# ergodicio/tsadar

Measured on AMD Instinct MI355X. Metric: spectra/sec (fwd+grad), 1024-lambda EPW+IAW form factor, batch 4096, higher is better.
Workload: dtype f64

## Files before the change

tsadar_amd/csrc/k_spectrum_fused.inc:

```

#ifdef TSFF_TRACE
__device__ unsigned long long* g_trace_buf = nullptr;
#define TSFF_STAMP(k) do { if (tid == 0 && g_trace_buf) g_trace_buf[(size_t)item * 16 + (k)] = wall_clock64(); } while (0)
#define TSFF_STAMP_WAVE(k) do { if (lane == 0 && g_trace_buf) g_trace_buf[(size_t)item * 16 + (k) + hw] = wall_clock64(); } while (0)
#define TSFF_STAMP_HW() do { if (tid == 0 && g_trace_buf) g_trace_buf[(size_t)item * 16] = ((unsigned long long)__builtin_amdgcn_s_getreg(20 | (31 << 11)) << 32) | (unsigned)__builtin_amdgcn_s_getreg(4 | (31 << 11)); } while (0)
#else
#define TSFF_STAMP(k) do {} while (0)
#define TSFF_STAMP_WAVE(k) do {} while (0)
#define TSFF_STAMP_HW() do {} while (0)
#endif

constexpr int kRedSums = 32;
template <int NI, int GM, bool ZH, bool EX = false>
__global__ __launch_bounds__(kHalf, 2) void k_spectrum_fused(KStatic S, KCall K, int f0, int flags,
                                                             const double* __restrict__ lrec) {
  const bool use_ks = flags & kFlagKsCache, interleaved = flags & kFlagInterleaved;
  const int item = blockIdx.x;
  const int f_il = interleaved ? (int)(item >= K.B) : 0;
  const int b = K.b0 + item - f_il * K.B, tid = threadIdx.x;
  const size_t gitem = (size_t)f_il * K.Btot + b;
  constexpr int TPF = kHalf, NW = TPF / 64;
  constexpr bool PAD = kSelectFree<NI>;
  const int ht = tid, lane = tid & 63, hw = tid >> 6;
  const int f = __builtin_amdgcn_readfirstlane(interleaved ? f_il : f0);
  extern __shared__ __align__(16) unsigned char smem[];
  TSFF_STAMP_HW();
  TSFF_STAMP(1);
  const Smem m = carve(smem, S, 1, GM, use_ks, true, ZH, EX);
  constexpr int NPk = TSFF_NP(NI);
  const double* __restrict__ xpar = K.params + (size_t)b * S.NP;
  const int npts = S.npts, NA = S.n_angles;
  const int hs = S.hs, Ls = npts / 4 + 2 * hs;
  double* xs = m.x;
  auto XA = [&](int j) { return (j & 3) * Ls + (j >> 2) + hs; };
  Tables T;
  const double lam_shift = S.lam_shift[f];
  const double* __restrict__ omgs = S.omgs[f];
  const int jp[2] = {kPair * ht, npts / 2 + kPair * ht};
  double ws[2][kPair + 1];
  LineS<NI> L;
  double* __restrict__ ksc = use_ks ? m.ksc : nullptr;
  {
    TSFF_STAGE_LOCALS;
    stage_issue(TSFF_STAGE_ARGS, m, S, K, S.shared_fe ? 0 : b, ZH, f);
    stage_commit(TSFF_STAGE_ARGS, m, S, K, S.shared_fe ? 0 : b, T, ZH, f, PAD);
#pragma unroll
    for (int p = 0; p < 2; ++p)
#pragma unroll
      for (int q = 0; q <= kPair; ++q) ws[p][q] = omgs[min(jp[p] + q, npts - 1)];
    {
      lines_load<NI>(lrec + gitem * kLineRec, 1, [](double v) { return uni(v); }, L);
    }
    if (use_ks) ks_cache_fill(ksc, jp, ws, L.wpe2, npts);
    zero_phase_halos(xs, Ls, hs, ht, TPF);
  }
  double w_lo[2], w_hi[2];
#pragma unroll
  for (int p = 0; p < 2; ++p) {
    w_lo[p] = lane_f64(ws[p][0], 0);
    w_hi[p] = lane_f64(ws[p][kPair], 63);
  }
  const bool far0 = far_range_w<NI>(w_lo[0], w_hi[0], L), far1 = far_range_w<NI>(w_lo[1], w_hi[1], L);
  const double ex_wse = ((lane >> 4) & 1) ? w_hi[1] : w_hi[0];
  __syncthreads();
  TSFF_STAMP(2);
  auto JQ = [&](int q) { return jp[q >> 1] + (q & 1); };
  LineS<NI> J[kStrip];
  KsAcc KA[kStrip];
  double xa[kStrip];
#pragma unroll
  for (int q = 0; q < kStrip; ++q) { zero_lines<NI>(J[q]); xa[q] = 0.0; KA[q].p1a = KA[q].p2a = KA[q].p1b = KA[q].p2b = 0.0; }
  const double cw = -0.5 * L.i2wL * L.i2wL;
  double* exb = m.ex;
  if (EX) {
    const int Pb = (lane >> 4) & 1, ab = lane & 15;
    if (lane < 32 && ab < NA) unit_boundary_fill<NI, PAD>(ex_wse, m.cosa[ab], L, T, exb + 16 * (2 * hw + Pb) + ab);
    __builtin_amdgcn_fence(__ATOMIC_RELEASE, "wavefront");
    __builtin_amdgcn_wave_barrier();
    __builtin_amdgcn_fence(__ATOMIC_ACQUIRE, "wavefront");
  }
  cdouble_t* arp = (cdouble_t*)(lrec + (size_t)K.Btot * (interleaved ? 2 : 1) * kLineRec + gitem * 2 * (size_t)NA);
  auto sweep = [&](auto pair_tag, auto far_tag) {
    constexpr int P = decltype(pair_tag)::value;
    constexpr bool FAR = decltype(far_tag)::value;
    const int jb = jp[P];
    const int j2 = min(jb + kPair, npts - 1);
    const double ks2 = EX ? (use_ks ? ksc[j2] : ks_eval(ws[P][kPair], L.wpe2)) : 0.0;
    cdouble_t* pn = arp;
    double ct_n = pn[0], wa_n = pn[1];
    const double* exu = EX ? exb + 16 * (2 * hw + P) : nullptr;
    double ksa = 0.0, ksb = 0.0;
    if constexpr (kSweepSched<NI, GM, ZH, EX>) {
      ksa = use_ks ? ksc[jb] : ks_eval(ws[P][0], L.wpe2);
      ksb = use_ks ? ksc[min(jb + 1, npts - 1)] : ks_eval(ws[P][1], L.wpe2);
    }
    for (int a = 0; a < NA; ++a) {
      const double ct = ct_n, wa = wa_n;
      { pn += a + 1 < NA ? 2 : 0; ct_n = pn[0]; wa_n = pn[1]; }
      if constexpr (kSweepSched<NI, GM, ZH, EX>) {
        constexpr int q0 = kPair * P;
        static_assert(kPair == 2, "pair_step_sched is written out for two points");
        pair_step_sched<NI, GM, ZH, FAR, PAD>(ws[P], ksa, ksb, ks2, exu + a, pair_has_next<NI, P, 2>(1, jb + 1, npts), L, T, ct, wa, cw,
                                              xa[q0], J[q0], KA[q0], xa[q0 + 1], J[q0 + 1], KA[q0 + 1]);
        continue;
      }
      Base b0;
      base_eval<NI, PAD>(ws[P][0], use_ks ? ksc[jb] : ks_eval(ws[P][0], L.wpe2), ct, L, T, b0);
      const Base b0f = b0;
#pragma unroll
      for (int i = 0; i < kPair; ++i) {
        constexpr int q0 = kPair * P;
        const int q = q0 + i, j = jb + i;
        const bool has_next = pair_has_next<NI, P, 2>(i, j, npts);
        Base b1;
        if (EX && i == kPair - 1) {
          neighbour_take<NI>(b0f, exu + a, ks2, ct, L, b1);
        } else {
          base_eval<NI, PAD>(ws[P][i + 1], use_ks ? ksc[min(j + 1, npts - 1)] : ks_eval(ws[P][i + 1], L.wpe2), ct, L, T, b1);
        }
        row_step<NI, GM, ZH, FAR, PAD>(b0, b1, has_next, L, T, ct, wa, cw, xa[q], J[q], KA[q]);
        b0 = b1;
      }
    }
  };
  if (far0) sweep(std::integral_constant<int, 0>{}, std::true_type{}); else sweep(std::integral_constant<int, 0>{}, std::false_type{});
  if (far1) sweep(std::integral_constant<int, 1>{}, std::true_type{}); else sweep(std::integral_constant<int, 1>{}, std::false_type{});
  TSFF_STAMP_WAVE(9);
#pragma unroll
  for (int q = 0; q < kStrip; ++q) {
    const int j = JQ(q);
    const double ksa = use_ks ? ksc[j] : ks_eval(ws[q >> 1][q & 1], L.wpe2);
    const double ksb = use_ks ? ksc[min(j + 1, npts - 1)] : ks_eval(ws[q >> 1][(q & 1) + 1], L.wpe2);
    ks_columns<NI>(KA[q], ksa, ksb, L, J[q]);
  }
  {
    const bool filt = f == TSFF_FEATURE_ELE && S.filt;
#pragma unroll
    for (int q = 0; q < kStrip; ++q) store_scaled(xs + XA(JQ(q)), xa[q], ws[q >> 1][q & 1], filt, S.filt, JQ(q));
  }
  __syncthreads();
  TSFF_STAMP(3);

  constexpr int BPT = 4;
  const bool raw = S.raw[f];
  const size_t row4 = (size_t)b * TSFF_NBINS + 4 * ht;
  double dpre[BPT], npre[BPT], lpre[BPT];
  uint8_t mpre[BPT];
#pragma unroll
  for (int r = 0; r < BPT; ++r) {
    dpre[r] = K.data[f][row4 + r];
    npre[r] = K.noise[f] ? K.noise[f][row4 + r] : 0.0;
    lpre[r] = f == TSFF_FEATURE_ELE ? S.lam_bin[f][4 * ht + r] : 0.0;
    mpre[r] = S.mask[f][4 * ht + r];
  }
  const double amps = raw ? 1.0 : K.amps[f][b];
  const double* __restrict__ lrp = lrec + gitem * kLineRec + 9 + 4 * NI;
  const double p_lam_v = lrp[0], p_amp1_v = lrp[1], p_amp2_v = lrp[2], p_amp3_v = lrp[3];
  double wpre[BPT];
  {
    const bool filt = f == TSFF_FEATURE_ELE && S.filt;
#pragma unroll
    for (int r = 0; r < BPT; ++r) {
      const double w = omgs[4 * ht + r];
      wpre[r] = filt ? w * w * S.filt[4 * ht + r] : w * w;
    }
  }
  double ybin[BPT] = {0.0, 0.0, 0.0, 0.0};
  conv4_phase<1>(xs, Ls, ht + S.cf_a0[f] + hs, (cdouble_t*)(S.ptaps[f] + S.cf_i0[f]), S.cf_na[f], ybin);
  double M = ybin[0];
  int pstar = 4 * ht;
#pragma unroll
  for (int r = 1; r < BPT; ++r)
    if (ybin[r] > M) { M = ybin[r]; pstar = 4 * ht + r; }
  half_argmax<NW>(M, pstar, m.red, 0, hw, lane);
  TSFF_STAMP(4);
  const double invM = raw ? 1.0 : 1.0 / M;
  const double p_lam = uni(p_lam_v), p_amp1 = uni(p_amp1_v), p_amp2 = uni(p_amp2_v), p_amp3 = uni(p_amp3_v);
  double Tb[BPT], Ap[BPT];
  double s0 = 0.0, s1 = 0.0;
#pragma unroll
  for (int r = 0; r < BPT; ++r) {
    const int pb = 4 * ht + r;
    const double A = bin_amplitude(f, raw, amps, lpre[r], p_lam, p_amp1, p_amp2, p_amp3);
    Ap[r] = A;
    const double t = thry_value(A, ybin[r], invM, K.noise[f] != nullptr, npre[r]);
    if (K.thry[f]) K.thry[f][(size_t)b * TSFF_NBINS + pb] = t;
    Tb[r] = bin_loss(S, K, f, dpre[r], t, mpre[r], s0, s1);
  }

  double sn = 0.0, a1b = 0.0, a2b = 0.0;
#pragma unroll
  for (int r = 0; r < BPT; ++r) norm_adjoint_bin(f, Tb[r], ybin[r], invM, Ap[r], amps, lpre[r], p_lam, sn, a1b, a2b);
  {
    double v5[5] = {s0, s1, sn, a1b, a2b};
#pragma unroll
    for (int k = 0; k < 5; ++k) v5[k] = wave_sum(v5[k]);
    if (lane == 0) {
#pragma unroll
      for (int k = 0; k < 5; ++k) m.red[kRedSums + k * NW + hw] = v5[k];
    }
  }
#pragma unroll
  for (int r = 0; r < BPT; ++r) xs[XA(4 * ht + r)] = Tb[r] * Ap[r] * invM;
  __syncthreads();
  TSFF_STAMP(5);
  double sx[4] = {0.0, 0.0, 0.0, 0.0};
  conv4_phase<-1>(xs, Ls, ht + S.ca_a0[f] + hs, (cdouble_t*)(S.ptaps[f] + S.ca_i0[f]), S.ca_na[f], sx);

  __syncthreads();
  TSFF_STAMP(6);
  {
    const double* r = m.red + kRedSums;
    s0 = (r[0] + r[1]) + (r[2] + r[3]);
    s1 = (r[NW] + r[NW + 1]) + (r[NW + 2] + r[NW + 3]);
    sn = (r[2 * NW] + r[2 * NW + 1]) + (r[2 * NW + 2] + r[2 * NW + 3]);
    a1b = (r[3 * NW] + r[3 * NW + 1]) + (r[3 * NW + 2] + r[3 * NW + 3]);
    a2b = (r[4 * NW] + r[4 * NW + 1]) + (r[4 * NW + 2] + r[4 * NW + 3]);
  }
  if (ht == 0) {
    if (f == TSFF_FEATURE_ELE) { K.lpart[(size_t)b * 3 + 1] = s0; K.lpart[(size_t)b * 3 + 2] = s1; }
    else K.lpart[(size_t)b * 3 + 0] = s0;
  }
  if (raw) sn = a1b = a2b = 0.0;
  {
    const bool filt = f == TSFF_FEATURE_ELE && S.filt;
    const double cn = sn * invM;
    const int s_first = 4 * ht - pstar - S.toff[f], nt = S.ntaps[f];
#pragma unroll
    for (int r = 0; r < 4; ++r) {
      const int i = 4 * ht + r, st = s_first + r;
      const double xb = (st >= 0 && st < nt) ? __builtin_fma(-cn, m.taps[3 + st], sx[r]) : sx[r];
      xs[XA(i)] = xb * wpre[r];
    }
  }
  __syncthreads();
  constexpr int NLB = 9 + 3 * NI;
  LineS<NI> LB;
  zero_lines<NI>(LB);
#pragma unroll
  for (int q = 0; q < kStrip; ++q) {
    const double xb = xs[XA(JQ(q))];
    LB.wpe2 += xb * J[q].wpe2; LB.wL += xb * J[q].wL; LB.kL += xb * J[q].kL; LB.ivTe += xb * J[q].ivTe;
    LB.a_e += xb * J[q].a_e; LB.Ud += xb * J[q].Ud; LB.Vd += xb * J[q].Vd; LB.m += xb * J[q].m;
    LB.pref += xb * xa[q];
#pragma unroll
    for (int s = 0; s < NI; ++s) { LB.ixi[s] += xb * J[q].ixi[s]; LB.a_i[s] += xb * J[q].a_i[s]; LB.cs[s] += xb * J[q].cs[s]; }
  }
  LB.pref *= 1.0 / L.pref;
#pragma unroll
  for (int s = 0; s < NI; ++s) LB.a_i[s] *= -0.5;
  {
    double lb[kLBRec];
    lines_adj_store<NI>(LB, lb);
#pragma unroll
    for (int k = 0; k < NLB; ++k) lb[k] = wave_sum(lb[k]);
    lb[NLB] = a1b; lb[NLB + 1] = a2b;
    const size_t nitems = (size_t)K.Btot * (interleaved ? 2 : 1);
    double mine = 0.0;
#pragma unroll
    for (int k = 0; k < NLB + 2; ++k) mine = lane == k ? lb[k] : mine;
    if (lane < NLB + 2) K.lbrec[((size_t)lane * NW + hw) * nitems + gitem] = mine;
  }
  TSFF_STAMP(8);
}

template <int NI>
__global__ __launch_bounds__(64) void k_fused_prep(KStatic S, const double* __restrict__ params, int B, int f0, int nload,
                                                   double* __restrict__ lrec, double* __restrict__ finrec, double* __restrict__ arec) {
  constexpr int NPk = TSFF_NP(NI);
  const int item = blockIdx.x * 64 + threadIdx.x;
  if (item >= B * nload) return;
  const size_t nitems = (size_t)B * nload;
  const int l = item / B, b = item - l * B, f = nload == 2 ? l : f0;
  const double* __restrict__ x = params + (size_t)b * S.NP;
  double sgv[NPk];
#pragma unroll
  for (int s = 0; s < NPk; ++s) sgv[s] = S.p_sig[s] ? sigmoid(x[s]) : 0.0;
  Phys<NI> p;
  load_phys<NI>(x, S.p_scale, S.p_shift, S.p_sig, S.ti_same, true, p, sgv);
  LineS<NI> L;
  make_lines<NI>(p, S.lam_shift[f], 0, 1, L);
  {
    double ph[NPk + 1];
    phys_to_array<NI>(p, ph);
    double* __restrict__ q = finrec + item;
#pragma unroll
    for (int k = 0; k <= NPk; ++k) q[(size_t)k * nitems] = ph[k];
#pragma unroll
    for (int k = 0; k < NPk; ++k) q[(size_t)(NPk + 1 + k) * nitems] = sgv[k];
    lines_store<NI>(L, q + (size_t)(2 * NPk + 1) * nitems, nitems);
  }
  double* __restrict__ r = lrec + (size_t)item * kLineRec;
  lines_store<NI>(L, r, 1);
  r[9 + 4 * NI] = p.lam; r[10 + 4 * NI] = p.amp1; r[11 + 4 * NI] = p.amp2; r[12 + 4 * NI] = p.amp3;
  if (arec) {
    double2* __restrict__ ar = reinterpret_cast<double2*>(arec) + (size_t)item * S.n_angles;
    for (int a = 0; a < S.n_angles; ++a) ar[a] = make_double2(S.cos_sa[a], S.w_sa[a] * L.pref);
  }
}

template <int NI>
__global__ __launch_bounds__(kThreads) void k_fused_finish(KStatic S, const double* __restrict__ finrec, const double* __restrict__ lbrec,
                                                     const double* __restrict__ lpart, int B, int f0, int nload, int gm,
                                                     const uint8_t* __restrict__ gmask, double* __restrict__ grad,
                                                     double* __restrict__ loss_out, const int* __restrict__ act, int n_act,
                                                     long B_global, long b_off, double* __restrict__ packed) {
  constexpr int NPk = TSFF_NP(NI), NLB = 9 + 3 * NI, NW = kHalf / 64;
  __shared__ double red[8];
  const int lane = threadIdx.x;
  const int per_wg = kThreads / nload;
  if (blockIdx.x == gridDim.x - 1) {
    double a[3] = {0.0, 0.0, 0.0};
    constexpr int U = 8;
    for (int b0 = threadIdx.x; b0 < B; b0 += U * kThreads) {
      double v[U][3];
#pragma unroll
      for (int u = 0; u < U; ++u) {
        const int bb = b0 + u * kThreads;
#pragma unroll
        for (int k = 0; k < 3; ++k) v[u][k] = bb < B ? lpart[(size_t)bb * 3 + k] : 0.0;
      }
#pragma unroll
      for (int u = 0; u < U; ++u)
        if (b0 + u * kThreads < B) { a[0] += v[u][0]; a[1] += v[u][1]; a[2] += v[u][2]; }
    }
    double* out = packed ? packed : loss_out;
    for (int k = 0; k < 3; ++k) {
      const double v = block_sum(a[k], red);
      if (threadIdx.x == 0) out[k] = v;
    }
    return;
  }
  const int b = blockIdx.x * per_wg + lane / nload, l = nload == 2 ? (lane & 1) : 0;
  int actv[NPk];
#pragma unroll
  for (int k = 0; k < NPk; ++k) actv[k] = (packed && k < n_act) ? act[k] : -1;
  const size_t nitems = (size_t)B * nload;
  double gv[NPk];
#pragma unroll
  for (int s = 0; s < NPk; ++s) gv[s] = 0.0;
  if (b < B) {
    const int f = nload == 2 ? l : f0;
    const size_t item = (size_t)l * B + b;
    const double* __restrict__ q = finrec + item;
    double ph[NPk + 1], sgv[NPk];
#pragma unroll
    for (int k = 0; k <= NPk; ++k) ph[k] = q[(size_t)k * nitems];
#pragma unroll
    for (int k = 0; k < NPk; ++k) sgv[k] = q[(size_t)(NPk + 1 + k) * nitems];
    Phys<NI> p;
    phys_from_lds<NI>(ph, p);
    q += (size_t)(2 * NPk + 1) * nitems;
    LineS<NI> L;
    lines_load<NI>(q, nitems, [](double v) { return v; }, L);
    double lb[NLB];
#pragma unroll
    for (int k = 0; k < NLB; ++k) {
      const double* __restrict__ r = lbrec + (size_t)k * NW * nitems + item;
      lb[k] = (r[0] + r[nitems]) + (r[2 * nitems] + r[3 * nitems]);
    }
    const double a1b = lbrec[(size_t)NLB * NW * nitems + item], a2b = lbrec[(size_t)(NLB + 1) * NW * nitems + item];
    LineS<NI> LB;
    zero_lines<NI>(LB);
    lines_adj_load<NI>(lb, true, LB);
    double g[NPk];
#pragma unroll
    for (int s = 0; s < NPk; ++s) g[s] = 0.0;
    make_lines_adjoint<NI>(p, S.lam_shift[f], 0, 1, L, LB, g);
    amp_adjoint(f, a1b, a2b, g);
    tie_renorm_adjoint<NI>(S, p, gm == 1, g);
#pragma unroll
    for (int s = 0; s < NPk; ++s) gv[s] = activation_adjoint(g[s], S.p_scale[s], S.p_sig[s], [&] { return sgv[s]; }, gmask[s]);
  }
  if (nload == 2) {
#pragma unroll
    for (int s = 0; s < NPk; ++s) {
      const double o = __shfl_xor(gv[s], 1, 64);
      gv[s] = (lane & 1) ? 0.0 : gv[s] + o;
    }
  }
  if (b < B && l == 0) {
    if (packed) {
#pragma unroll
      for (int k = 0; k < NPk; ++k) {
        double v = 0.0;
#pragma unroll
        for (int s = 0; s < NPk; ++s) v = actv[k] == s ? gv[s] : v;
        if (actv[k] >= 0) packed[3 + (size_t)k * B_global + b_off + b] = v;
      }
    } else {
#pragma unroll
      for (int s = 0; s < NPk; ++s) grad[(size_t)b * NPk + s] = gv[s];
    }
  }
  if (packed) {
    const long n = (long)n_act * B_global;
    if ((long)B < B_global)
      for (long i = (long)blockIdx.x * kThreads + lane; i < n; i += (long)(gridDim.x - 1) * kThreads) {
        const long k = i / B_global, bl = i - k * B_global - b_off;
        if (bl < 0 || bl >= B) packed[3 + i] = 0.0;
      }
  }
}
```

tsadar_amd/csrc/tsff_device.h:

```cpp
#pragma once
#include <hip/hip_runtime.h>
#include <stdint.h>
#include <type_traits>

#include "../../include/tsff.h"

namespace tsff {

constexpr int kThreads = 256;
constexpr int kStrip = 4;
constexpr int kNP_MAX = TSFF_NP(TSFF_MAX_ION);

enum SpectrumFlag : int {
  kFlagAccumulate = 1,
  kFlagKsCache = 2,
  kFlagInterleaved = 4,
  kFlagOwnScalars = 8,
  kFlagSplit = 16,
};

constexpr double kC = 2.99792458e10;
constexpr double kMe = 510.9896 / (kC * kC);
constexpr double kMp = kMe * 1836.1;
constexpr double kRe = 2.8179e-13;
constexpr double kPi = 3.14159265358979323846;
constexpr double kEsq = kMe * kC * kC * kRe;
constexpr double kC0sq = 4.0 * kPi * kEsq / kMe;
constexpr double kOmgLnum = 2.0 * kPi * 1e7 * kC;
constexpr double kInvSqrt2Pi = 0.39894228040143267794;
constexpr double kSqrt2 = 1.41421356237309504880;

constexpr double kXi2_0 = -8.2;
constexpr double kXi2_h = 0.01;
constexpr double kXi2_ih = 100.0;
constexpr int kNXi2 = TSFF_NXI2;
constexpr int kNXi1 = TSFF_NXI1;

#ifndef TSFF_NEWTON
#define TSFF_NEWTON 1
#endif
__device__ __forceinline__ double frcp(double x) {
  double y = __builtin_amdgcn_rcp(x);
  double e = __builtin_fma(-x, y, 1.0);
  y = __builtin_fma(y, e, y);
#if TSFF_NEWTON > 1
  e = __builtin_fma(-x, y, 1.0);
  y = __builtin_fma(y, e, y);
#endif
  return y;
}

__device__ __forceinline__ void fsqrt2(double x, double& s, double& is) {
  const double y = __builtin_amdgcn_rsq(x);
  double g = x * y, h = 0.5 * y;
  double r = __builtin_fma(-h, g, 0.5);
  g = __builtin_fma(g, r, g);
  h = __builtin_fma(h, r, h);
#if TSFF_NEWTON > 1
  r = __builtin_fma(-h, g, 0.5);
  g = __builtin_fma(g, r, g);
  h = __builtin_fma(h, r, h);
#endif
  const double d = __builtin_fma(-g, g, x);
  s = __builtin_fma(d, h, g);
  is = h + h;
}

__device__ __forceinline__ void fsqrt2_pair(double x0, double x1, double& s0, double& is0, double& s1, double& is1) {
  static_assert(TSFF_NEWTON == 1, "fsqrt2_pair is written out for one refinement step");
  const double y0 = __builtin_amdgcn_rsq(x0), y1 = __builtin_amdgcn_rsq(x1);
  __builtin_amdgcn_sched_barrier(0);
  double g0 = x0 * y0, g1 = x1 * y1, h0 = 0.5 * y0, h1 = 0.5 * y1;
  __builtin_amdgcn_sched_barrier(0);
  const double r0 = __builtin_fma(-h0, g0, 0.5), r1 = __builtin_fma(-h1, g1, 0.5);
  __builtin_amdgcn_sched_barrier(0);
  g0 = __builtin_fma(g0, r0, g0); g1 = __builtin_fma(g1, r1, g1);
  h0 = __builtin_fma(h0, r0, h0); h1 = __builtin_fma(h1, r1, h1);
  __builtin_amdgcn_sched_barrier(0);
  const double d0 = __builtin_fma(-g0, g0, x0), d1 = __builtin_fma(-g1, g1, x1);
  __builtin_amdgcn_sched_barrier(0);
  s0 = __builtin_fma(d0, h0, g0); s1 = __builtin_fma(d1, h1, g1);
  is0 = h0 + h0; is1 = h1 + h1;
}

__device__ __forceinline__ double uni(double x) {
  const int lo = __builtin_amdgcn_readfirstlane(__double2loint(x));
  const int hi = __builtin_amdgcn_readfirstlane(__double2hiint(x));
  return __hiloint2double(hi, lo);
}

__device__ __forceinline__ double next_lane_f64(double v, double last) {
  constexpr int kWaveShl1 = 0x130;
  const int lo = __builtin_amdgcn_update_dpp(__double2loint(last), __double2loint(v), kWaveShl1, 0xf, 0xf, false);
  const int hi = __builtin_amdgcn_update_dpp(__double2hiint(last), __double2hiint(v), kWaveShl1, 0xf, 0xf, false);
  return __hiloint2double(hi, lo);
}

__device__ __forceinline__ double wave_sum(double v) {
#pragma unroll
  for (int o = 32; o > 0; o >>= 1) v += __shfl_xor(v, o, 64);
  return v;
}

__device__ __forceinline__ double block_sum(double v, double* scratch) {
  v = wave_sum(v);
  const int lane = threadIdx.x & 63, w = threadIdx.x >> 6;
  __syncthreads();
  if (lane == 0) scratch[w] = v;
  __syncthreads();
  return (scratch[0] + scratch[1]) + (scratch[2] + scratch[3]);
}

__device__ __forceinline__ void block_argmax(double& v, int& idx, double* scratch) {
#pragma unroll
  for (int o = 32; o > 0; o >>= 1) {
    double ov = __shfl_xor(v, o, 64);
    int oi = __shfl_xor(idx, o, 64);
    if (ov > v || (ov == v && oi < idx)) { v = ov; idx = oi; }
  }
  const int lane = threadIdx.x & 63, w = threadIdx.x >> 6;
  __syncthreads();
  if (lane == 0) { scratch[w] = v; scratch[4 + w] = (double)idx; }
  __syncthreads();
  v = scratch[0]; idx = (int)scratch[4];
#pragma unroll
  for (int k = 1; k < 4; ++k) {
    double ov = scratch[k]; int oi = (int)scratch[4 + k];
    if (ov > v || (ov == v && oi < idx)) { v = ov; idx = oi; }
  }
}

struct Tables {
  const double2* zp;
  const double* W;
  const double2* ht;
  const double2* hc;
  const double2* hcm;
  const double* Wm;
  double* Wb;
  double* Hy;
  double* Hs;
  double vx0, dv, idv, vxlast;
  double u0, utop;
  double uhi;
  const double* etab;
  int nvx;
};
__device__ __forceinline__ void tables_set_grid(Tables& T, double vx0, double dv, int nvx) {
  T.vx0 = vx0; T.dv = dv; T.idv = 1.0 / dv; T.vxlast = vx0 + (nvx - 1) * dv; T.nvx = nvx;
  T.u0 = -vx0 * T.idv; T.utop = (double)(nvx - 1) * (1.0 - 1.1102230246251565e-16); T.uhi = (double)(nvx - 1);
}

struct FeAcc {
  int iw, ih;
  double w0, w1, y0, y1, s0, s1;
};
__device__ __forceinline__ void fe_acc_init(FeAcc& a) { a.iw = a.ih = -1; a.w0 = a.w1 = a.y0 = a.y1 = a.s0 = a.s1 = 0.0; }
__device__ __forceinline__ void fe_flush_w(FeAcc& a, double* Wb) {
  if (a.iw >= 0) { atomicAdd(&Wb[a.iw], a.w0); atomicAdd(&Wb[a.iw + 1], a.w1); }
  a.w0 = a.w1 = 0.0;
}
__device__ __forceinline__ void fe_flush_h(FeAcc& a, double* Hy, double* Hs) {
  if (a.ih >= 0) {
    atomicAdd(&Hy[a.ih], a.y0); atomicAdd(&Hy[a.ih + 1], a.y1);
    atomicAdd(&Hs[a.ih], a.s0); atomicAdd(&Hs[a.ih + 1], a.s1);
  }
  a.y0 = a.y1 = a.s0 = a.s1 = 0.0;
}
__device__ __forceinline__ void fe_add_w(FeAcc& a, double* Wb, double xe, double wb) {
  const double xlast = kXi2_0 + (kNXi2 - 1) * kXi2_h;
  const double u = (xe - kXi2_0) * kXi2_ih;
  int i = (int)u;
  i = i < 0 ? 0 : (i > kNXi2 - 2 ? kNXi2 - 2 : i);
  double t = (xe - (kXi2_0 + i * kXi2_h)) * kXi2_ih;
  t = xe < kXi2_0 ? 0.0 : (xe > xlast ? 1.0 : t);
  if (i != a.iw) { fe_flush_w(a, Wb); a.iw = i; }
  a.w0 += wb * (1.0 - t);
  a.w1 += wb * t;
}
__device__ __forceinline__ void fe_add_h(FeAcc& a, const Tables& T, double x, double hb) {
  if (x < T.vx0 || x > T.vxlast) return;
  const double u = (x - T.vx0) * T.idv;
  int i = (int)u;
  i = i < 0 ? 0 : (i > T.nvx - 2 ? T.nvx - 2 : i);
  const double t = (x - (T.vx0 + i * T.dv)) * T.idv;
  if (i != a.ih) { fe_flush_h(a, T.Hy, T.Hs); a.ih = i; }
  const double t2 = t * t, t3 = t2 * t;
  a.y0 += hb * (2.0 * t3 - 3.0 * t2 + 1.0);
  a.y1 += hb * (3.0 * t2 - 2.0 * t3);
  a.s0 += hb * (t3 - 2.0 * t2 + t) * T.dv;
  a.s1 += hb * (t3 - t2) * T.dv;
}

struct WCell { double a, b, t; bool in; };
__device__ __forceinline__ void w_request(const double* W, double xe, WCell& c) {
#pragma clang fp contract(off)
  constexpr double kTop = (double)(kNXi2 - 1) * (1.0 - 1.1102230246251565e-16);
  const double u = __builtin_fma(xe, kXi2_ih, -kXi2_0 * kXi2_ih);
  const double uc = fmin(fmax(u, 0.0), kTop);
  const double fl = __builtin_floor(uc);
  c.t = uc - fl;
  const int i = (int)fl;
  c.a = W[i]; c.b = W[i + 1];
  c.in = u == uc;
}
__device__ __forceinline__ void w_finish(const WCell& c, double& w, double& dw) {
#pragma clang fp contract(off)
  const double d = c.b - c.a;
  w = __builtin_fma(c.t, d, c.a);
  dw = c.in ? d * kXi2_ih : 0.0;
}
__device__ __forceinline__ void w_lookup(const double* W, double xe, double& w, double& dw) {
  WCell c;
  w_request(W, xe, c);
  w_finish(c, w, dw);
}

__device__ __forceinline__ void hermite_coeffs(double2 a, double2 b, double dv, double2& c01, double2& c23) {
  const double f0 = a.x, f1 = b.x, m0 = a.y * dv, m1 = b.y * dv;
  c01 = make_double2(f0, m0);
  c23 = make_double2(-3.0 * f0 + 3.0 * f1 - 2.0 * m0 - m1, 2.0 * f0 - 2.0 * f1 + m0 + m1);
}

__device__ __forceinline__ void hermite_pad_cell(double2* hc, int nvx, double outside, int tid) {
  if (tid == 0) { hc[2 * (nvx - 1)] = make_double2(outside, 0.0); hc[2 * (nvx - 1) + 1] = make_double2(0.0, 0.0); }
}

struct HCell { double2 c01, c23; double t; bool out; };
template <bool PAD = false>
__device__ __forceinline__ void hermite_request(const Tables& T, double x, HCell& c) {
#pragma clang fp contract(off)
  const double u = __builtin_fma(x, T.idv, T.u0);
  const double uc = PAD ? fmin(fmax(u, -1.0), T.uhi) : fmin(fmax(u, 0.0), T.utop);
  const double fl = __builtin_floor(uc);
  c.t = uc - fl;
  int i = (int)fl;
  if (PAD) { const unsigned iu = (unsigned)i, itop = (unsigned)(T.nvx - 1); i = (int)(iu < itop ? iu : itop); }
  c.c01 = T.hc[2 * i]; c.c23 = T.hc[2 * i + 1];
  c.out = !PAD && u != uc;
}
__device__ __forceinline__ void hermite_finish(const Tables& T, const HCell& c, double& H, double& dH) {
#pragma clang fp contract(off)
  const double t = c.t;
  const double Hi = __builtin_fma(t, __builtin_fma(t, __builtin_fma(t, c.c23.y, c.c23.x), c.c01.y), c.c01.x);
  const double dHi = __builtin_fma(t, __builtin_fma(3.0 * t, c.c23.y, 2.0 * c.c23.x), c.c01.y) * T.idv;
  H = c.out ? -50.0 : Hi;
  dH = c.out ? 0.0 : dHi;
}
template <bool PAD = false>
__device__ __forceinline__ void hermite_lookup_c(const Tables& T, double x, double& H, double& dH) {
  HCell c;
  hermite_request<PAD>(T, x, c);
  hermite_finish(T, c, H, dH);
}

__device__ __forceinline__ void hermite_lookup(const Tables& T, double x, double& H, double& dH) {
  double u = (x - T.vx0) * T.idv;
  int i = (int)u;
  i = i < 0 ? 0 : (i > T.nvx - 2 ? T.nvx - 2 : i);
  const double t = (x - (T.vx0 + i * T.dv)) * T.idv;
  const double2 a = T.ht[i], b = T.ht[i + 1];
  const double f0 = a.x, f1 = b.x, m0 = a.y * T.dv, m1 = b.y * T.dv;
  const double c2 = -3.0 * f0 + 3.0 * f1 - 2.0 * m0 - m1;
  const double c3 = 2.0 * f0 - 2.0 * f1 + m0 + m1;
  if (x < T.vx0 || x > T.vxlast) { H = -50.0; dH = 0.0; }
  else {
    H = f0 + t * (m0 + t * (c2 + t * c3));
    dH = (m0 + t * (2.0 * c2 + 3.0 * t * c3)) * T.idv;
  }
}

template <int NI>
struct Phys {
  double Te, ne, m, lam, amp1, amp2, amp3, neg, teg, ud, Va;
  double Ti[NI], Z[NI], A[NI], fr[NI];
  double fsum;
};

template <int NI>
struct LineS {
  double wpe2, wL, kL, ivTe, a_e, pref, Ud, Vd;
  double i2wL;
  double m;
  double ixi[NI], a_i[NI], cs[NI];
  double hai[NI];
};

__device__ __forceinline__ double grad_coef(int g, int G) {
  return G == 1 ? -1.0 / 200.0 : -1.0 / 200.0 + (double)g / (100.0 * (double)(G - 1));
}

template <int NI>
__device__ __forceinline__ void make_lines(const Phys<NI>& p, double lam_shift, int g, int G, LineS<NI>& L) {
  const double cg = grad_coef(g, G);
  const double ne_g = 1.0e20 * p.ne * (1.0 + p.neg * cg);
  const double Te_g = p.Te * (1.0 + p.teg * cg);
  L.wL = kOmgLnum / (p.lam + lam_shift);
  L.i2wL = 2.0 / L.wL;
  L.m = 0.0;
  L.wpe2 = kC0sq * ne_g;
  L.kL = sqrt(L.wL * L.wL - L.wpe2) / kC;
  L.ivTe = 1.0 / sqrt(Te_g / kMe);
  L.a_e = L.wpe2 * L.ivTe * L.ivTe;
  L.pref = kRe * kRe * ne_g / (2.0 * kPi * kC);
  L.Ud = p.ud * 1e6;
  L.Vd = p.Va * 1e6;
  double Zbar = 0.0;
#pragma unroll
  for (int s = 0; s < NI; ++s) Zbar += p.Z[s] * p.fr[s];
#pragma unroll
  for (int s = 0; s < NI; ++s) {
    const double Ms = p.A[s] * kMp;
    const double vTi = sqrt(p.Ti[s] / Ms);
    L.ixi[s] = 1.0 / (kSqrt2 * vTi);
    L.a_i[s] = kC0sq * kMe * p.Z[s] * p.Z[s] * p.fr[s] * ne_g / (Zbar * p.Ti[s]);
    L.cs[s] = p.fr[s] * p.Z[s] * p.Z[s] / (Zbar * vTi);
    L.hai[s] = -0.5 * L.a_i[s];
  }
}

template <int NI>
__device__ __forceinline__ void make_lines_uniform(const Phys<NI>& p, double lam_shift, int g, int G, LineS<NI>& L) {
  make_lines<NI>(p, lam_shift, g, G, L);
  L.wpe2 = uni(L.wpe2); L.wL = uni(L.wL); L.i2wL = uni(L.i2wL); L.kL = uni(L.kL); L.ivTe = uni(L.ivTe);
  L.a_e = uni(L.a_e); L.pref = uni(L.pref); L.Ud = uni(L.Ud); L.Vd = uni(L.Vd);
#pragma unroll
  for (int s = 0; s < NI; ++s) { L.ixi[s] = uni(L.ixi[s]); L.a_i[s] = uni(L.a_i[s]); L.cs[s] = uni(L.cs[s]); L.hai[s] = uni(L.hai[s]); }
}

template <int NI>
__device__ __forceinline__ void make_lines_adjoint(const Phys<NI>& p, double lam_shift, int g, int G,
                                                   const LineS<NI>& L, const LineS<NI>& LB, double* pb) {
  const double cg = grad_coef(g, G);
  const double gfn = 1.0 + p.neg * cg, gft = 1.0 + p.teg * cg;
  const double ne_g = 1.0e20 * p.ne * gfn;
  const double Te_g = p.Te * gft;
  double wpe2b = LB.wpe2, wLb = LB.wL, ivTeb = LB.ivTe;
  double ne_gb = LB.pref * (kRe * kRe / (2.0 * kPi * kC));
  wpe2b += LB.a_e * L.ivTe * L.ivTe;
  ivTeb += LB.a_e * 2.0 * L.wpe2 * L.ivTe;
  wLb += LB.kL * L.wL / (kC * kC * L.kL);
  wpe2b += LB.kL * (-0.5 / (kC * kC * L.kL));
  double Zbar = 0.0;
#pragma unroll
  for (int s = 0; s < NI; ++s) Zbar += p.Z[s] * p.fr[s];
  double Zbarb = 0.0;
#pragma unroll
  for (int s = 0; s < NI; ++s) {
    const double Ms = p.A[s] * kMp;
    const double vTi = sqrt(p.Ti[s] / Ms);
    const double Z2 = p.Z[s] * p.Z[s];
    double Tib = 0.0, Zb = 0.0, frb = 0.0;
    const double ai_over_fr = kC0sq * kMe * Z2 * ne_g / (Zbar * p.Ti[s]);
    Zb += LB.a_i[s] * 2.0 * L.a_i[s] / p.Z[s];
    frb += LB.a_i[s] * ai_over_fr;
    ne_gb += LB.a_i[s] * L.a_i[s] / ne_g;
    Zbarb -= LB.a_i[s] * L.a_i[s] / Zbar;
    Tib -= LB.a_i[s] * L.a_i[s] / p.Ti[s];
    Tib += LB.ixi[s] * (-0.5 * L.ixi[s] / p.Ti[s]);
    Tib += LB.cs[s] * (-0.5 * L.cs[s] / p.Ti[s]);
    Zb += LB.cs[s] * 2.0 * L.cs[s] / p.Z[s];
    frb += LB.cs[s] * Z2 / (Zbar * vTi);
    Zbarb -= LB.cs[s] * L.cs[s] / Zbar;
    pb[TSFF_P_ION0 + 4 * s + TSFF_ION_TI] += Tib;
    pb[TSFF_P_ION0 + 4 * s + TSFF_ION_Z] += Zb;
    pb[TSFF_P_ION0 + 4 * s + TSFF_ION_FRACT] += frb;
  }
#pragma unroll
  for (int s = 0; s < NI; ++s) {
    pb[TSFF_P_ION0 + 4 * s + TSFF_ION_Z] += Zbarb * p.fr[s];
    pb[TSFF_P_ION0 + 4 * s + TSFF_ION_FRACT] += Zbarb * p.Z[s];
  }
  const double Te_gb = ivTeb * (-0.5 * L.ivTe / Te_g);
  ne_gb += wpe2b * kC0sq;
  const double lam0 = p.lam + lam_shift;
  pb[TSFF_P_LAM] += wLb * (-L.wL / lam0);
  pb[TSFF_P_NE] += ne_gb * 1.0e20 * gfn;
  pb[TSFF_P_NE_GRADIENT] += ne_gb * 1.0e20 * p.ne * cg;
  pb[TSFF_P_TE] += Te_gb * gft;
  pb[TSFF_P_TE_GRADIENT] += Te_gb * p.Te * cg;
  pb[TSFF_P_UD] += LB.Ud * 1e6;
  pb[TSFF_P_VA] += LB.Vd * 1e6;
  pb[TSFF_P_M] += LB.m;
}


template <bool CLAMP = true>
__device__ __forceinline__ double fexp(double x) {
  if (CLAMP) x = fmax(x, -800.0);
  const double n = __builtin_rint(x * 1.4426950408889634074);
  double r = __builtin_fma(n, -6.93147180369123816490e-01, x);
  r = __builtin_fma(n, -1.90821492927058770002e-10, r);
  double p = 1.6059043836821613e-10;
  p = __builtin_fma(p, r, 2.08767569878681e-09);
  p = __builtin_fma(p, r, 2.505210838544172e-08);
  p = __builtin_fma(p, r, 2.755731922398589e-07);
  p = __builtin_fma(p, r, 2.7557319223985893e-06);
  p = __builtin_fma(p, r, 2.48015873015873e-05);
  p = __builtin_fma(p, r, 1.984126984126984e-04);
  p = __builtin_fma(p, r, 1.388888888888889e-03);
  p = __builtin_fma(p, r, 8.333333333333333e-03);
  p = __builtin_fma(p, r, 4.1666666666666664e-02);
  p = __builtin_fma(p, r, 1.6666666666666666e-01);
  p = __builtin_fma(p, r, 0.5);
// ... 556 lines not shown
```

Before: 5.332 million.

## Use scatter-style multi-value wave reductions and reload omega to ease register pressure

Replaces the per-value butterfly wave_sum loops with a recursive halving scatter reduction. Each exchange step sums two values into one using permlane32/16 swaps and DPP, so each lane ends up owning one final sum, with the -0.5 and 1/pref scaling folded into the first step. For the GM==1, NI==1, EX specialisation it also reloads the third omega point from global memory instead of keeping it live in registers across the sweep, and adds asm barriers to stop the compiler from merging the copies. The aim is fewer shuffle instructions in the reductions and lower VGPR pressure, at the cost of extra global loads and more complex lane-ownership logic.

```diff
diff --git a/tsadar_amd/csrc/k_spectrum_fused.inc b/tsadar_amd/csrc/k_spectrum_fused.inc
--- a/tsadar_amd/csrc/k_spectrum_fused.inc
+++ b/tsadar_amd/csrc/k_spectrum_fused.inc
@@ -20,6 +20,7 @@
   const int b = K.b0 + item - f_il * K.B, tid = threadIdx.x;
   const size_t gitem = (size_t)f_il * K.Btot + b;
   constexpr int TPF = kHalf, NW = TPF / 64;
+  constexpr bool kLeanKs = GM == 1 && NI == 1 && EX;
   constexpr bool PAD = kSelectFree<NI>;
   const int ht = tid, lane = tid & 63, hw = tid >> 6;
   const int f = __builtin_amdgcn_readfirstlane(interleaved ? f_il : f0);
@@ -51,7 +52,16 @@
     {
       lines_load<NI>(lrec + gitem * kLineRec, 1, [](double v) { return uni(v); }, L);
     }
-    if (use_ks) ks_cache_fill(ksc, jp, ws, L.wpe2, npts);
+    if constexpr (kLeanKs) {
+      double wsc[2][kPair + 1];
+#pragma unroll
+      for (int p = 0; p < 2; ++p)
+#pragma unroll
+        for (int q = 0; q <= kPair; ++q) { wsc[p][q] = ws[p][q]; asm volatile("" : "+v"(wsc[p][q])); }
+      if (use_ks) ks_cache_fill(ksc, jp, wsc, L.wpe2, npts);
+    } else {
+      if (use_ks) ks_cache_fill(ksc, jp, ws, L.wpe2, npts);
+    }
     zero_phase_halos(xs, Ls, hs, ht, TPF);
   }
   double w_lo[2], w_hi[2];
@@ -60,6 +70,12 @@
     w_lo[p] = lane_f64(ws[p][0], 0);
     w_hi[p] = lane_f64(ws[p][kPair], 63);
   }
+  auto w_third = [&](int p) {
+    const double* o = omgs;
+    int t = ht;
+    asm volatile("" : "+s"(o), "+v"(t));
+    return o[min(kPair * t + p * (npts / 2) + kPair, npts - 1)];
+  };
   const bool far0 = far_range_w<NI>(w_lo[0], w_hi[0], L), far1 = far_range_w<NI>(w_lo[1], w_hi[1], L);
   const double ex_wse = ((lane >> 4) & 1) ? w_hi[1] : w_hi[0];
   __syncthreads();
@@ -85,7 +101,13 @@
     constexpr bool FAR = decltype(far_tag)::value;
     const int jb = jp[P];
     const int j2 = min(jb + kPair, npts - 1);
-    const double ks2 = EX ? (use_ks ? ksc[j2] : ks_eval(ws[P][kPair], L.wpe2)) : 0.0;
+    double wr[kPair + 1];
+    if constexpr (kLeanKs) {
+#pragma unroll
+      for (int q = 0; q <= kPair; ++q) wr[q] = q == kPair ? w_third(P) : ws[P][q];
+    }
+    const double (&wP)[kPair + 1] = [&]() -> const double (&)[kPair + 1] { if constexpr (kLeanKs) return wr; else return ws[P]; }();
+    const double ks2 = EX ? (use_ks ? ksc[j2] : ks_eval(wP[kPair], L.wpe2)) : 0.0;
     cdouble_t* pn = arp;
     double ct_n = pn[0], wa_n = pn[1];
     const double* exu = EX ? exb + 16 * (2 * hw + P) : nullptr;
@@ -105,7 +127,7 @@
         continue;
       }
       Base b0;
-      base_eval<NI, PAD>(ws[P][0], use_ks ? ksc[jb] : ks_eval(ws[P][0], L.wpe2), ct, L, T, b0);
+      base_eval<NI, PAD>(wP[0], use_ks ? ksc[jb] : ks_eval(wP[0], L.wpe2), ct, L, T, b0);
       const Base b0f = b0;
 #pragma unroll
       for (int i = 0; i < kPair; ++i) {
@@ -116,7 +138,7 @@
         if (EX && i == kPair - 1) {
           neighbour_take<NI>(b0f, exu + a, ks2, ct, L, b1);
         } else {
-          base_eval<NI, PAD>(ws[P][i + 1], use_ks ? ksc[min(j + 1, npts - 1)] : ks_eval(ws[P][i + 1], L.wpe2), ct, L, T, b1);
+          base_eval<NI, PAD>(wP[i + 1], use_ks ? ksc[min(j + 1, npts - 1)] : ks_eval(wP[i + 1], L.wpe2), ct, L, T, b1);
         }
         row_step<NI, GM, ZH, FAR, PAD>(b0, b1, has_next, L, T, ct, wa, cw, xa[q], J[q], KA[q]);
         b0 = b1;
@@ -126,17 +148,25 @@
   if (far0) sweep(std::integral_constant<int, 0>{}, std::true_type{}); else sweep(std::integral_constant<int, 0>{}, std::false_type{});
   if (far1) sweep(std::integral_constant<int, 1>{}, std::true_type{}); else sweep(std::integral_constant<int, 1>{}, std::false_type{});
   TSFF_STAMP_WAVE(9);
+  double wl[2][kPair + 1];
+  if constexpr (kLeanKs) {
+#pragma unroll
+    for (int p = 0; p < 2; ++p)
+#pragma unroll
+      for (int q = 0; q <= kPair; ++q) wl[p][q] = q == kPair ? w_third(p) : ws[p][q];
+  }
+  const double (&wq)[2][kPair + 1] = [&]() -> const double (&)[2][kPair + 1] { if constexpr (kLeanKs) return wl; else return ws; }();
 #pragma unroll
   for (int q = 0; q < kStrip; ++q) {
     const int j = JQ(q);
-    const double ksa = use_ks ? ksc[j] : ks_eval(ws[q >> 1][q & 1], L.wpe2);
-    const double ksb = use_ks ? ksc[min(j + 1, npts - 1)] : ks_eval(ws[q >> 1][(q & 1) + 1], L.wpe2);
+    const double ksa = use_ks ? ksc[j] : ks_eval(wq[q >> 1][q & 1], L.wpe2);
+    const double ksb = use_ks ? ksc[min(j + 1, npts - 1)] : ks_eval(wq[q >> 1][(q & 1) + 1], L.wpe2);
     ks_columns<NI>(KA[q], ksa, ksb, L, J[q]);
   }
   {
     const bool filt = f == TSFF_FEATURE_ELE && S.filt;
 #pragma unroll
-    for (int q = 0; q < kStrip; ++q) store_scaled(xs + XA(JQ(q)), xa[q], ws[q >> 1][q & 1], filt, S.filt, JQ(q));
+    for (int q = 0; q < kStrip; ++q) store_scaled(xs + XA(JQ(q)), xa[q], wq[q >> 1][q & 1], filt, S.filt, JQ(q));
   }
   __syncthreads();
   TSFF_STAMP(3);
@@ -192,13 +222,11 @@
 #pragma unroll
   for (int r = 0; r < BPT; ++r) norm_adjoint_bin(f, Tb[r], ybin[r], invM, Ap[r], amps, lpre[r], p_lam, sn, a1b, a2b);
   {
-    double v5[5] = {s0, s1, sn, a1b, a2b};
-#pragma unroll
-    for (int k = 0; k < 5; ++k) v5[k] = wave_sum(v5[k]);
-    if (lane == 0) {
-#pragma unroll
-      for (int k = 0; k < 5; ++k) m.red[kRedSums + k * NW + hw] = v5[k];
-    }
+    const double v5[5] = {s0, s1, sn, a1b, a2b};
+    const double v = wave_sums_scatter<5>(v5, lane);
+    bool own;
+    const int k = scatter_lane<5>(lane, own);
+    if (own) m.red[kRedSums + k * NW + hw] = v;
   }
 #pragma unroll
   for (int r = 0; r < BPT; ++r) xs[XA(4 * ht + r)] = Tb[r] * Ap[r] * invM;
@@ -246,20 +274,20 @@
 #pragma unroll
     for (int s = 0; s < NI; ++s) { LB.ixi[s] += xb * J[q].ixi[s]; LB.a_i[s] += xb * J[q].a_i[s]; LB.cs[s] += xb * J[q].cs[s]; }
   }
-  LB.pref *= 1.0 / L.pref;
-#pragma unroll
-  for (int s = 0; s < NI; ++s) LB.a_i[s] *= -0.5;
   {
     double lb[kLBRec];
     lines_adj_store<NI>(LB, lb);
-#pragma unroll
-    for (int k = 0; k < NLB; ++k) lb[k] = wave_sum(lb[k]);
-    lb[NLB] = a1b; lb[NLB + 1] = a2b;
+    double lbs[NLB], lbc[NLB];
+    constexpr unsigned scaled = (1u << 5) | (1u << 9) | (NI > 1 ? 1u << 12 : 0u);
+#pragma unroll
+    for (int k = 0; k < NLB; ++k) { lbs[k] = lb[k]; lbc[k] = k == 5 ? 1.0 / L.pref : ((scaled >> k) & 1u) ? -0.5 : 1.0; }
+    double mine = wave_sums_scatter_scaled<NLB, scaled>(lbs, lbc, lane);
+    bool own;
+    int k = scatter_lane<NLB>(lane, own);
+    if (lane == 1) { mine = a1b; k = NLB; }
+    if (lane == 2) { mine = a2b; k = NLB + 1; }
     const size_t nitems = (size_t)K.Btot * (interleaved ? 2 : 1);
-    double mine = 0.0;
-#pragma unroll
-    for (int k = 0; k < NLB + 2; ++k) mine = lane == k ? lb[k] : mine;
-    if (lane < NLB + 2) K.lbrec[((size_t)lane * NW + hw) * nitems + gitem] = mine;
+    if (own || lane == 1 || lane == 2) K.lbrec[((size_t)k * NW + hw) * nitems + gitem] = mine;
   }
   TSFF_STAMP(8);
 }
diff --git a/tsadar_amd/csrc/tsff_device.h b/tsadar_amd/csrc/tsff_device.h
--- a/tsadar_amd/csrc/tsff_device.h
+++ b/tsadar_amd/csrc/tsff_device.h
@@ -4,6 +4,7 @@
 #include <type_traits>
 
 #include "../../include/tsff.h"
+#include "wave_scatter.h"
 
 namespace tsff {
 
@@ -100,6 +101,92 @@
 #pragma unroll
   for (int o = 32; o > 0; o >>= 1) v += __shfl_xor(v, o, 64);
   return v;
+}
+
+template <int O>
+__device__ __forceinline__ double scatter_exchange_add(double lo, double hi, int lane) {
+  static_assert(O == 32 || O == 16 || O == 8 || O == 4, "offsets 2 and 1 never scatter");
+  if constexpr (O >= 16) {
+    const unsigned a0 = __double2loint(lo), a1 = __double2hiint(lo), b0 = __double2loint(hi), b1 = __double2hiint(hi);
+    if constexpr (O == 32) {
+      const auto r0 = __builtin_amdgcn_permlane32_swap(a0, b0, false, false), r1 = __builtin_amdgcn_permlane32_swap(a1, b1, false, false);
+      return __hiloint2double(r1[0], r0[0]) + __hiloint2double(r1[1], r0[1]);
+    } else {
+      const auto r0 = __builtin_amdgcn_permlane16_swap(a0, b0, false, false), r1 = __builtin_amdgcn_permlane16_swap(a1, b1, false, false);
+      return __hiloint2double(r1[0], r0[0]) + __hiloint2double(r1[1], r0[1]);
+    }
+  } else {
+    const bool up = lane & O;
+    return (up ? hi : lo) + __shfl_xor(up ? lo : hi, O, 64);
+  }
+}
+
+template <int O>
+__device__ __forceinline__ double xor_lane_f64(double v) {
+  if constexpr (O == 8 || O == 2 || O == 1) {
+    constexpr int ctrl = O == 8 ? 0x128 : O == 2 ? 0x4E : 0xB1;
+    const int lo = __builtin_amdgcn_mov_dpp(__double2loint(v), ctrl, 0xf, 0xf, false);
+    const int hi = __builtin_amdgcn_mov_dpp(__double2hiint(v), ctrl, 0xf, 0xf, false);
+    return __hiloint2double(hi, lo);
+  } else {
+    return __shfl_xor(v, O, 64);
+  }
+}
+
+template <int N, int O>
+__device__ __forceinline__ double wave_sums_scatter_step(const double (&w)[N], int lane) {
+  if constexpr (O == 0) {
+    static_assert(N == 1, "one value per lane is left behind the last offset");
+    return w[0];
+  } else if constexpr (N > 1) {
+    constexpr int H = (N + 1) / 2;
+    double u[H];
+#pragma unroll
+    for (int i = 0; i < H; ++i) u[i] = scatter_exchange_add<O>(w[i], H + i < N ? w[H + i] : 0.0, lane);
+    return wave_sums_scatter_step<H, O / 2>(u, lane);
+  } else {
+    double u[1];
+    if constexpr (O >= 16) u[0] = scatter_exchange_add<O>(w[0], w[0], lane);
+    else u[0] = w[0] + xor_lane_f64<O>(w[0]);
+    return wave_sums_scatter_step<1, O / 2>(u, lane);
+  }
+}
+
+template <int N>
+__device__ __forceinline__ double wave_sums_scatter(const double (&v)[N], int lane) {
+  static_assert(N >= 1 && N <= kScatterMax, "one value per group of four lanes at most");
+  return wave_sums_scatter_step<N, 32>(v, lane);
+}
+
+template <int N, unsigned SCALED>
+__device__ __forceinline__ double wave_sums_scatter_scaled(const double (&v)[N], const double (&c)[N], int lane) {
+  static_assert(N >= 2 && N <= kScatterMax && SCALED < (1u << N), "one value per group of four lanes at most; the offset 32 must scatter");
+  constexpr int H = (N + 1) / 2;
+  double u[H];
+#pragma unroll
+  for (int i = 0; i < H; ++i) {
+    const double lo = v[i], hi = H + i < N ? v[H + i] : 0.0;
+    const bool slo = (SCALED >> i) & 1u, shi = H + i < N && ((SCALED >> (H + i)) & 1u);
+    if (slo || shi) {
+      const double cc = (lane & 32) ? (shi ? c[H + i < N ? H + i : i] : 1.0) : (slo ? c[i] : 1.0);
+      const auto r0 = __builtin_amdgcn_permlane32_swap(__double2loint(lo), __double2loint(hi), false, false);
+      const auto r1 = __builtin_amdgcn_permlane32_swap(__double2hiint(lo), __double2hiint(hi), false, false);
+      const double lower = __hiloint2double(r1[0], r0[0]), upper = __hiloint2double(r1[1], r0[1]);
+      u[i] = __builtin_fma(lower, cc, upper * cc);
+    } else {
+      u[i] = scatter_exchange_add<32>(lo, hi, lane);
+    }
+  }
+  return wave_sums_scatter_step<H, 16>(u, lane);
+}
+
+template <int N>
+__device__ __forceinline__ int scatter_lane(int lane, bool& own) {
+  constexpr uint64_t values = scatter_values(N);
+  constexpr uint32_t valid = scatter_valid(N);
+  const int g = lane >> 2;
+  own = (lane & 3) == 0 && ((valid >> g) & 1u);
+  return (int)(values >> (4 * g)) & 15;
 }
 
 __device__ __forceinline__ double block_sum(double v, double* scratch) {
diff --git a/tsadar_amd/csrc/wave_scatter.h b/tsadar_amd/csrc/wave_scatter.h
--- /dev/null
+++ b/tsadar_amd/csrc/wave_scatter.h
@@ -0,0 +1,42 @@
+#pragma once
+#include <cstdint>
+
+namespace tsff {
+
+constexpr int kScatterMax = 16;
+
+constexpr int scatter_value_of_lane(int N, int lane) {
+  int off = 0, size = N, n = N;
+  for (int o = 32; o >= 4 && n > 1; o >>= 1) {
+    const int h = (n + 1) / 2;
+    if (lane & o) { off += h; size = size > h ? size - h : 0; }
+    else size = size < h ? size : h;
+    n = h;
+  }
+  return size > 0 ? off : -1;
+}
+
+constexpr int scatter_exchanges(int N) {
+  int n = N, c = 0;
+  for (int o = 32; o >= 1; o >>= 1) {
+    if (o >= 4 && n > 1) n = (n + 1) / 2;
+    c += n;
+  }
+  return c;
+}
+
+constexpr uint64_t scatter_values(int N) {
+  uint64_t t = 0;
+  for (int g = 0; g < 16; ++g) {
+    const int k = scatter_value_of_lane(N, 4 * g);
+    t |= (uint64_t)(k < 0 ? 0 : k) << (4 * g);
+  }
+  return t;
+}
+constexpr uint32_t scatter_valid(int N) {
+  uint32_t m = 0;
+  for (int g = 0; g < 16; ++g) m |= (uint32_t)(scatter_value_of_lane(N, 4 * g) >= 0) << g;
+  return m;
+}
+
+}
```

Result: faster. 5.500 million, median of 6 (+3.1%).
